# bastienjacquet/CudaDepthMapIntegration

Hardware: AMD Instinct MI355X
Metric: Gvoxel-projections/s (higher is better)
Workload: dtype f64

## Files before the change

### cudadepthmapintegration_amd/csrc/fusion_tile.hip

```cpp
#include <stdlib.h>

#include <algorithm>
#include <type_traits>

#include "fusion_kernels.h"
#include "fusion_device.h"

#ifndef DMI_T1_CHAINS
#define DMI_T1_CHAINS 4
#endif
#ifndef DMI_T1_COLUMN_CHAINS
#define DMI_T1_COLUMN_CHAINS 2
#endif
#if !defined(DMI_TUNING) && (defined(DMI_EXP_SKIP_WINDOW_VIEWS) || defined(DMI_EXP_SAME_REC) || defined(DMI_EXP_NO_WINDOW_LOADS) || \
                             defined(DMI_EXP_NO_LANE_MARGIN))
#error "a DMI_EXP_* switch that changes results was defined without DMI_TUNING"
#endif

namespace dmi {

int tile_shape_index(int variant);

namespace {

// ... 586 lines not shown
          f32x2 v;
          v.x = __uint_as_float(R[q]);
          v.y = __uint_as_float(R[q + 1]);
          asm volatile("" : "+v"(v));
          return v;
        };
        const f32x2 Bwi = pk_fnma_slo(O, pair_of(8), vec_of(2));
        const f32x2 Bwj = pk_fnma_slo(O, pair_of(10), vec_of(4));
        const f32x2 DH = pk_fnma_slo(O, pair_of(12), vec_of(6));
#ifdef DMI_WINPAIR_LANE_HELD
        const f32x2 H0 = pk_fma_hi0_vv(LJ, Bwj, pk_fma_lo0_vs(LJ, Bwi, A2));
#else
        const f32x2 H0 = pk_fma_hi0_vv(LJ, Bwj, pk_fma_lo0_vv(LJ, Bwi, A2));
#endif
        f32x2 CA;
        CA.x = acz;
        CA.y = __builtin_fmaf(acz, __uint_as_float(R[15]), -__uint_as_float(R[14]));
        const f32x2 C0 = pk_fma_hi0_sv(LJ, pair_of(10), pk_fma_lo0_sv(LJ, pair_of(8), CA));
        const f32x2 DC = vec_of(12);
        unsigned long long M2 = (0x4B400000ull + (unsigned)kWinAnchorX) | ((0x4B400000ull + (unsigned)kWinAnchorY) << 32);
        asm volatile("" : "+s"(M2));
        float magic_v = 0x1.8p23f + (float)(4 * kWinAnchorY);
        asm volatile("" : "+v"(magic_v));
        auto first_voxel = [&](double &hxf, double &hyf, double &czf64) __attribute__((always_inline)) {
          const kernarg_t kf = KFRESH();
          const TileMapRec *rf = kf->tile_maps + m;
          double wxf = wx, wyf = wy, wzf = wz0;
          if constexpr (ROT) {
            const czvec4 b = cload(reinterpret_cast<const czvec4 *>(kf->cz_table + (int64_t)k0 * 4));
            wxf = (wx + b[0]) + kf->g[3], wyf = (wy + b[1]) + kf->g[7], wzf = (wz0 + b[2]) + kf->g[11];
            czf64 = ((cload(&rf->rz0) * wxf + cload(&rf->rz1) * wyf) + cload(&kf->maps[m].rt[10]) * wzf) + cload(&rf->rz3);
          } else {
            czf64 = ((cload(&rf->rz0) * wx + cload(&rf->rz1) * wy) + cload(kf->cz_table + (int64_t)m * kf->kpad + k0)) + cload(&rf->rz3);
          }
          hxf = __builtin_fma(cload(&rf->cpx), wxf, __builtin_fma(cload(&rf->cpy), wyf, __builtin_fma(cload(&rf->cpz), wzf, cload(&rf->cp0))));
          hyf = __builtin_fma(cload(&rf->cqx), wxf, __builtin_fma(cload(&rf->cqy), wyf, __builtin_fma(cload(&rf->cqz), wzf, cload(&rf->cq0))));
        };
        uint32_t undecided = 0, und_kk = 0;
        uint32_t window = 0;
        constexpr int WG = 4;
#ifdef DMI_T1_RCP_EVERY_VOXEL
        constexpr bool kNewton = false;
#else
        constexpr bool kNewton = true;
#endif
        [[maybe_unused]] f32x2 r_below;
        uint32_t pw[WG], pc[WG];
        auto consume = [&](int g0) __attribute__((always_inline)) {
          __builtin_amdgcn_s_waitcnt(0xc07f);
          if ((und_kk >> g0) & ((1u << WG) - 1u)) {
  #pragma unroll
            for (int q = 0; q < WG; ++q) pw[q] &= ((undecided >> (g0 + q)) & 1u) - 1u;
          }
  #pragma unroll
          for (int q = 0; q < WG; ++q) {
            int mbit;
            asm("v_bfe_i32 %0, %1, %2, 1" : "=v"(mbit) : "v"(pw[q]), "v"(pc[q]));
            acc_fma_vs<BASE, TK>(g0 + q, __hiloint2double(mbit & 0x3ff00000, 0), free_space);
          }
        };
  #pragma unroll
        for (int g0 = 0; g0 < TK; g0 += WG) {
          uint32_t wg[WG], cg[WG];
          mask_t m_und[WG];
          constexpr int IL = DMI_T1_CHAINS;
          if constexpr (kNewton) {
            static_assert(WG == 4, "the link order below is written for groups of four");
            f32x2 h[WG], cth[WG], r[WG], rpm[WG], rp[WG], t[WG];
            float tw[WG], mx[WG];
            auto kbits = [](int kk) __attribute__((always_inline)) { return (unsigned long long)(unsigned)__float_as_int((float)kk); };
            auto lz = [&](int u) __attribute__((always_inline)) { cth[u] = g0 + u > 0 ? ordered::pk_fma_s(kbits(g0 + u), DC, C0) : C0; };
            auto lh = [&](int u) __attribute__((always_inline)) { h[u] = g0 + u > 0 ? ordered::pk_fma_s(kbits(g0 + u), DH, H0) : H0; };
            auto l2 = [&](int u) __attribute__((always_inline)) {
              if (g0 + u > 0) tw[u] = ordered::two_minus(cth[u].x, u > 0 ? r[u > 0 ? u - 1 : 0].x : r_below.x);
            };
            auto lr = [&](int u) __attribute__((always_inline)) {
              r[u].x = g0 + u > 0 ? ordered::mul(u > 0 ? r[u > 0 ? u - 1 : 0].x : r_below.x, tw[u]) : ordered::rcp(cth[u].x);
            };
            auto lq = [&](int u) __attribute__((always_inline)) { rpm[u] = ordered::pk_fma_lo_s(h[u], r[u], M2); };
            auto lp = [&](int u) __attribute__((always_inline)) { rp[u] = ordered::pk_sub_s(rpm[u], M2); };
            auto lt = [&](int u) __attribute__((always_inline)) { t[u] = ordered::pk_fnma_lo(rp[u], cth[u], h[u]); };
            auto lm = [&](int u) __attribute__((always_inline)) { mx[u] = ordered::max_abs(t[u].x, t[u].y); };
            lz(0), lz(1), lz(2), lz(3);
            l2(0), lh(0), lr(0), lh(1), l2(1), lh(2), lr(1), lq(0), l2(2), lp(0), lr(2), lq(1), l2(3), lt(0), lr(3), lh(3);
            lp(1), lq(2), lm(0), lq(3), lt(1), lp(2), lm(1), lp(3), lt(2), lt(3), lm(2), lm(3);
            r_below = r[WG - 1];
  #pragma unroll
            for (int u = 0; u < WG; ++u) {
              m_und[u] = ballot(!(mx[u] < cth[u].y));
// ... 41 lines not shown
          if (m_und_any) {
  #pragma unroll
            for (int q = 0; q < WG; ++q) {
              if (m_und[q]) {
                or_where(undecided, m_und[q], 1u << (g0 + q));
                und_kk |= 1u << (g0 + q);
              }
            }
          }
          if (g0 == 0)
            window = __builtin_amdgcn_alignbit(w_hi, w_lo, (unsigned)x0p & 31u);
          else
            consume(g0 - WG);
  #pragma unroll
          for (int q = 0; q < WG; ++q) {
            pw[q] = (uint32_t)__builtin_amdgcn_ds_bpermute((int)wg[q], (int)window);
            pc[q] = cg[q];
          }
        }
        consume(TK - WG);
#ifndef DMI_NO_WINREC_PREFETCH
        asm volatile("s_waitcnt lgkmcnt(0)" : "+s"(next_rec));
#endif
#pragma unroll 1
        while (und_kk) {
#ifdef DMI_TUNING
          ++dbg_redo;
          ++dbg_win_redo;
#endif
          const int kk = __builtin_ctz(und_kk);
          und_kk &= und_kk - 1;
          const bool mine = (undecided >> kk) & 1u;
          const kernarg_t k2 = KFRESH();
          const TileMapRec *r2 = k2->tile_maps + m;
          double hxf, hyf, czf64;
          first_voxel(hxf, hyf, czf64);
          const double kd = (double)kk;
          const double hxk = __builtin_fma(kd, cload(&r2->cdhx), hxf), hyk = __builtin_fma(kd, cload(&r2->cdhy), hyf);
          double cz2;
          if constexpr (ROT) {
            const czvec4 b = cload(reinterpret_cast<const czvec4 *>(k2->cz_table + (int64_t)(k0 + kk) * 4));
            const double wxk = (wx + b[0]) + k2->g[3], wyk = (wy + b[1]) + k2->g[7], wzk = (wz0 + b[2]) + k2->g[11];
            cz2 = ((cload(&r2->rz0) * wxk + cload(&r2->rz1) * wyk) + cload(&k2->maps[m].rt[10]) * wzk) + cload(&r2->rz3);
          } else {
            cz2 = ((cload(&r2->rz0) * wx + cload(&r2->rz1) * wy) + cload(k2->cz_table + (int64_t)m * k2->kpad + k0 + kk)) + cload(&r2->rz3);
          }
// ... 5 lines not shown
          const double fu = ua2 - ru2, fv = va2 - rv2;
          const double chk = __builtin_fma(cload(&r2->cerrk), r, __builtin_fmax(__builtin_fabs(fu), __builtin_fabs(fv)));
          const bool p2 = mine && chk < 0.5 && __builtin_fabs(e0) < tiny;
          const int col = cvt_saturating(ru2) - x0c, row = cvt_saturating(rv2) - y0c;
          const uint32_t word = (uint32_t)__builtin_amdgcn_ds_bpermute(row << 2, (int)window);
          double val = free_space;
          bool hit = p2 && ((word >> (col & 31)) & 1u);
          const bool exact = mine && !p2;
          if (ballot(exact)) {
            const __amdgpu_buffer_rsrc_t rsrc =
                __builtin_amdgcn_make_buffer_rsrc(const_cast<void *>(cload(&r2->depth)), (short)0, k2->depth_bytes, 0x00020000);
            double ev = 0.0;
            const bool eh = exact ? tile_exact<DepthT>(KC(full), m, rsrc, i, j, k0 + kk, ev) : false;
            if (exact) {
              hit = eh;
              val = ev;
            }
          }
#pragma unroll
          for (int q = 0; q < TK; ++q) {
            if (kk == q) acc_add_v<BASE, TK>(q, ballot(hit), val);
          }
        }
        continue;
      }
    }
    const kernarg_t kv = KFRESH();
    const TileMapRec *rec = kv->tile_maps + m;
    const double *ct = kv->cz_table + (int64_t)m * kv->kpad + k0;
    double sz, rz3, hx, hy;
    [[maybe_unused]] f32x2 H0 = {0.f, 0.f}, C0 = {0.f, 0.f}, DH = {0.f, 0.f}, DC = {0.f, 0.f};
    double r20 = 0, r21 = 0, r22 = 0;
    [[maybe_unused]] double cz_first = 0, wxf = wx, wyf = wy, wzf = wz0;
    if constexpr (ROT) {
      sz = lane_ok ? cload(&rec->rz3) : -__builtin_inf();
      rz3 = 0;
      hx = hy = 0;
      if constexpr (T1) {
        const czvec4 b = cload(reinterpret_cast<const czvec4 *>(kv->cz_table + (int64_t)k0 * 4));
        wxf = (wx + b[0]) + KA(g)[3], wyf = (wy + b[1]) + KA(g)[7], wzf = (wz0 + b[2]) + KA(g)[11];
        cz_first = ((cload(&rec->rz0) * wxf + cload(&rec->rz1) * wyf) + cload(&kv->maps[m].rt[10]) * wzf) + sz;
      } else {
        r20 = cload(&rec->rz0);
        r21 = cload(&rec->rz1);
        r22 = cload(&kv->maps[m].rt[10]);
      }
// ... 652 lines not shown
```

### cudadepthmapintegration_amd/csrc/fusion_tile_acc.inc

```

template <int BASE, int TK>
__device__ __forceinline__ void acc_add_s(const int kk, mask_t m, double v ) {
  mask_t saved;
  switch (BASE + 2 * kk) {
    case 64: if constexpr (64 >= BASE && 64 < BASE + 2 * TK) asm volatile("s_and_saveexec_b64 %0, %1\n\tv_add_f64 v[64:65], v[64:65], %2\n\ts_mov_b64 exec, %0" : "=&s"(saved) : "s"(m), "s"(v) : "v64", "v65", "scc"); break;
    case 66: if constexpr (66 >= BASE && 66 < BASE + 2 * TK) asm volatile("s_and_saveexec_b64 %0, %1\n\tv_add_f64 v[66:67], v[66:67], %2\n\ts_mov_b64 exec, %0" : "=&s"(saved) : "s"(m), "s"(v) : "v66", "v67", "scc"); break;
    case 68: if constexpr (68 >= BASE && 68 < BASE + 2 * TK) asm volatile("s_and_saveexec_b64 %0, %1\n\tv_add_f64 v[68:69], v[68:69], %2\n\ts_mov_b64 exec, %0" : "=&s"(saved) : "s"(m), "s"(v) : "v68", "v69", "scc"); break;
    case 70: if constexpr (70 >= BASE && 70 < BASE + 2 * TK) asm volatile("s_and_saveexec_b64 %0, %1\n\tv_add_f64 v[70:71], v[70:71], %2\n\ts_mov_b64 exec, %0" : "=&s"(saved) : "s"(m), "s"(v) : "v70", "v71", "scc"); break;
    case 72: if constexpr (72 >= BASE && 72 < BASE + 2 * TK) asm volatile("s_and_saveexec_b64 %0, %1\n\tv_add_f64 v[72:73], v[72:73], %2\n\ts_mov_b64 exec, %0" : "=&s"(saved) : "s"(m), "s"(v) : "v72", "v73", "scc"); break;
    case 74: if constexpr (74 >= BASE && 74 < BASE + 2 * TK) asm volatile("s_and_saveexec_b64 %0, %1\n\tv_add_f64 v[74:75], v[74:75], %2\n\ts_mov_b64 exec, %0" : "=&s"(saved) : "s"(m), "s"(v) : "v74", "v75", "scc"); break;
    case 76: if constexpr (76 >= BASE && 76 < BASE + 2 * TK) asm volatile("s_and_saveexec_b64 %0, %1\n\tv_add_f64 v[76:77], v[76:77], %2\n\ts_mov_b64 exec, %0" : "=&s"(saved) : "s"(m), "s"(v) : "v76", "v77", "scc"); break;
    case 78: if constexpr (78 >= BASE && 78 < BASE + 2 * TK) asm volatile("s_and_saveexec_b64 %0, %1\n\tv_add_f64 v[78:79], v[78:79], %2\n\ts_mov_b64 exec, %0" : "=&s"(saved) : "s"(m), "s"(v) : "v78", "v79", "scc"); break;
    case 80: if constexpr (80 >= BASE && 80 < BASE + 2 * TK) asm volatile("s_and_saveexec_b64 %0, %1\n\tv_add_f64 v[80:81], v[80:81], %2\n\ts_mov_b64 exec, %0" : "=&s"(saved) : "s"(m), "s"(v) : "v80", "v81", "scc"); break;
    case 82: if constexpr (82 >= BASE && 82 < BASE + 2 * TK) asm volatile("s_and_saveexec_b64 %0, %1\n\tv_add_f64 v[82:83], v[82:83], %2\n\ts_mov_b64 exec, %0" : "=&s"(saved) : "s"(m), "s"(v) : "v82", "v83", "scc"); break;
    case 84: if constexpr (84 >= BASE && 84 < BASE + 2 * TK) asm volatile("s_and_saveexec_b64 %0, %1\n\tv_add_f64 v[84:85], v[84:85], %2\n\ts_mov_b64 exec, %0" : "=&s"(saved) : "s"(m), "s"(v) : "v84", "v85", "scc"); break;
    case 86: if constexpr (86 >= BASE && 86 < BASE + 2 * TK) asm volatile("s_and_saveexec_b64 %0, %1\n\tv_add_f64 v[86:87], v[86:87], %2\n\ts_mov_b64 exec, %0" : "=&s"(saved) : "s"(m), "s"(v) : "v86", "v87", "scc"); break;
    case 88: if constexpr (88 >= BASE && 88 < BASE + 2 * TK) asm volatile("s_and_saveexec_b64 %0, %1\n\tv_add_f64 v[88:89], v[88:89], %2\n\ts_mov_b64 exec, %0" : "=&s"(saved) : "s"(m), "s"(v) : "v88", "v89", "scc"); break;
    case 90: if constexpr (90 >= BASE && 90 < BASE + 2 * TK) asm volatile("s_and_saveexec_b64 %0, %1\n\tv_add_f64 v[90:91], v[90:91], %2\n\ts_mov_b64 exec, %0" : "=&s"(saved) : "s"(m), "s"(v) : "v90", "v91", "scc"); break;
    case 92: if constexpr (92 >= BASE && 92 < BASE + 2 * TK) asm volatile("s_and_saveexec_b64 %0, %1\n\tv_add_f64 v[92:93], v[92:93], %2\n\ts_mov_b64 exec, %0" : "=&s"(saved) : "s"(m), "s"(v) : "v92", "v93", "scc"); break;
    case 94: if constexpr (94 >= BASE && 94 < BASE + 2 * TK) asm volatile("s_and_saveexec_b64 %0, %1\n\tv_add_f64 v[94:95], v[94:95], %2\n\ts_mov_b64 exec, %0" : "=&s"(saved) : "s"(m), "s"(v) : "v94", "v95", "scc"); break;
    case 96: if constexpr (96 >= BASE && 96 < BASE + 2 * TK) asm volatile("s_and_saveexec_b64 %0, %1\n\tv_add_f64 v[96:97], v[96:97], %2\n\ts_mov_b64 exec, %0" : "=&s"(saved) : "s"(m), "s"(v) : "v96", "v97", "scc"); break;
    case 98: if constexpr (98 >= BASE && 98 < BASE + 2 * TK) asm volatile("s_and_saveexec_b64 %0, %1\n\tv_add_f64 v[98:99], v[98:99], %2\n\ts_mov_b64 exec, %0" : "=&s"(saved) : "s"(m), "s"(v) : "v98", "v99", "scc"); break;
    case 100: if constexpr (100 >= BASE && 100 < BASE + 2 * TK) asm volatile("s_and_saveexec_b64 %0, %1\n\tv_add_f64 v[100:101], v[100:101], %2\n\ts_mov_b64 exec, %0" : "=&s"(saved) : "s"(m), "s"(v) : "v100", "v101", "scc"); break;
    case 102: if constexpr (102 >= BASE && 102 < BASE + 2 * TK) asm volatile("s_and_saveexec_b64 %0, %1\n\tv_add_f64 v[102:103], v[102:103], %2\n\ts_mov_b64 exec, %0" : "=&s"(saved) : "s"(m), "s"(v) : "v102", "v103", "scc"); break;
// ... 720 lines not shown
    case 154: if constexpr (154 >= BASE && 154 < BASE + 2 * TK) asm volatile("s_mov_b64 %[sx], exec\n\tv_add_f64 %[diff], %[cz], -%[d]\n\ts_mov_b64 %[sh], exec\n\tv_cmpx_lt_f64_e64 vcc, %[diff], -%[delta]\n\tv_add_f64 v[154:155], v[154:155], %[fs]\n\ts_mov_b64 exec, %[sh]\n\tv_cmpx_ngt_f64_e64 vcc, |%[diff]|, %[delta]\n\ts_cbranch_execz .Ldmi_pot_end_%=\n\tv_mul_f64 %[near], %[slope], %[diff]\n\ts_mov_b64 %[sh], exec\n\tv_cmpx_gt_f64_e64 vcc, %[diff], %[thick]\n\tv_mul_f64 %[near], %[rho], 1.0\n\ts_mov_b64 exec, %[sh]\n\tv_cmpx_lt_f64_e64 vcc, %[diff], -%[thick]\n\tv_mul_f64 %[near], %[rho], -1.0\n\ts_mov_b64 exec, %[sh]\n\tv_add_f64 v[154:155], v[154:155], %[near]\n\t.Ldmi_pot_end_%=:\n\ts_mov_b64 exec, %[sx]" : [diff] "=&v"(diff), [near] "=&v"(near), [sx] "=&s"(sx), [sh] "=&s"(sh) : [d] "v"(d), [cz] "v"(cz), [delta] "v"(delta), [thick] "v"(thick), [slope] "v"(slope), [fs] "s"(free_space), [rho] "s"(rho) : "v154", "v155", "vcc"); break;
    case 156: if constexpr (156 >= BASE && 156 < BASE + 2 * TK) asm volatile("s_mov_b64 %[sx], exec\n\tv_add_f64 %[diff], %[cz], -%[d]\n\ts_mov_b64 %[sh], exec\n\tv_cmpx_lt_f64_e64 vcc, %[diff], -%[delta]\n\tv_add_f64 v[156:157], v[156:157], %[fs]\n\ts_mov_b64 exec, %[sh]\n\tv_cmpx_ngt_f64_e64 vcc, |%[diff]|, %[delta]\n\ts_cbranch_execz .Ldmi_pot_end_%=\n\tv_mul_f64 %[near], %[slope], %[diff]\n\ts_mov_b64 %[sh], exec\n\tv_cmpx_gt_f64_e64 vcc, %[diff], %[thick]\n\tv_mul_f64 %[near], %[rho], 1.0\n\ts_mov_b64 exec, %[sh]\n\tv_cmpx_lt_f64_e64 vcc, %[diff], -%[thick]\n\tv_mul_f64 %[near], %[rho], -1.0\n\ts_mov_b64 exec, %[sh]\n\tv_add_f64 v[156:157], v[156:157], %[near]\n\t.Ldmi_pot_end_%=:\n\ts_mov_b64 exec, %[sx]" : [diff] "=&v"(diff), [near] "=&v"(near), [sx] "=&s"(sx), [sh] "=&s"(sh) : [d] "v"(d), [cz] "v"(cz), [delta] "v"(delta), [thick] "v"(thick), [slope] "v"(slope), [fs] "s"(free_space), [rho] "s"(rho) : "v156", "v157", "vcc"); break;
    case 158: if constexpr (158 >= BASE && 158 < BASE + 2 * TK) asm volatile("s_mov_b64 %[sx], exec\n\tv_add_f64 %[diff], %[cz], -%[d]\n\ts_mov_b64 %[sh], exec\n\tv_cmpx_lt_f64_e64 vcc, %[diff], -%[delta]\n\tv_add_f64 v[158:159], v[158:159], %[fs]\n\ts_mov_b64 exec, %[sh]\n\tv_cmpx_ngt_f64_e64 vcc, |%[diff]|, %[delta]\n\ts_cbranch_execz .Ldmi_pot_end_%=\n\tv_mul_f64 %[near], %[slope], %[diff]\n\ts_mov_b64 %[sh], exec\n\tv_cmpx_gt_f64_e64 vcc, %[diff], %[thick]\n\tv_mul_f64 %[near], %[rho], 1.0\n\ts_mov_b64 exec, %[sh]\n\tv_cmpx_lt_f64_e64 vcc, %[diff], -%[thick]\n\tv_mul_f64 %[near], %[rho], -1.0\n\ts_mov_b64 exec, %[sh]\n\tv_add_f64 v[158:159], v[158:159], %[near]\n\t.Ldmi_pot_end_%=:\n\ts_mov_b64 exec, %[sx]" : [diff] "=&v"(diff), [near] "=&v"(near), [sx] "=&s"(sx), [sh] "=&s"(sh) : [d] "v"(d), [cz] "v"(cz), [delta] "v"(delta), [thick] "v"(thick), [slope] "v"(slope), [fs] "s"(free_space), [rho] "s"(rho) : "v158", "v159", "vcc"); break;
    case 160: if constexpr (160 >= BASE && 160 < BASE + 2 * TK) asm volatile("s_mov_b64 %[sx], exec\n\tv_add_f64 %[diff], %[cz], -%[d]\n\ts_mov_b64 %[sh], exec\n\tv_cmpx_lt_f64_e64 vcc, %[diff], -%[delta]\n\tv_add_f64 v[160:161], v[160:161], %[fs]\n\ts_mov_b64 exec, %[sh]\n\tv_cmpx_ngt_f64_e64 vcc, |%[diff]|, %[delta]\n\ts_cbranch_execz .Ldmi_pot_end_%=\n\tv_mul_f64 %[near], %[slope], %[diff]\n\ts_mov_b64 %[sh], exec\n\tv_cmpx_gt_f64_e64 vcc, %[diff], %[thick]\n\tv_mul_f64 %[near], %[rho], 1.0\n\ts_mov_b64 exec, %[sh]\n\tv_cmpx_lt_f64_e64 vcc, %[diff], -%[thick]\n\tv_mul_f64 %[near], %[rho], -1.0\n\ts_mov_b64 exec, %[sh]\n\tv_add_f64 v[160:161], v[160:161], %[near]\n\t.Ldmi_pot_end_%=:\n\ts_mov_b64 exec, %[sx]" : [diff] "=&v"(diff), [near] "=&v"(near), [sx] "=&s"(sx), [sh] "=&s"(sh) : [d] "v"(d), [cz] "v"(cz), [delta] "v"(delta), [thick] "v"(thick), [slope] "v"(slope), [fs] "s"(free_space), [rho] "s"(rho) : "v160", "v161", "vcc"); break;
    case 162: if constexpr (162 >= BASE && 162 < BASE + 2 * TK) asm volatile("s_mov_b64 %[sx], exec\n\tv_add_f64 %[diff], %[cz], -%[d]\n\ts_mov_b64 %[sh], exec\n\tv_cmpx_lt_f64_e64 vcc, %[diff], -%[delta]\n\tv_add_f64 v[162:163], v[162:163], %[fs]\n\ts_mov_b64 exec, %[sh]\n\tv_cmpx_ngt_f64_e64 vcc, |%[diff]|, %[delta]\n\ts_cbranch_execz .Ldmi_pot_end_%=\n\tv_mul_f64 %[near], %[slope], %[diff]\n\ts_mov_b64 %[sh], exec\n\tv_cmpx_gt_f64_e64 vcc, %[diff], %[thick]\n\tv_mul_f64 %[near], %[rho], 1.0\n\ts_mov_b64 exec, %[sh]\n\tv_cmpx_lt_f64_e64 vcc, %[diff], -%[thick]\n\tv_mul_f64 %[near], %[rho], -1.0\n\ts_mov_b64 exec, %[sh]\n\tv_add_f64 v[162:163], v[162:163], %[near]\n\t.Ldmi_pot_end_%=:\n\ts_mov_b64 exec, %[sx]" : [diff] "=&v"(diff), [near] "=&v"(near), [sx] "=&s"(sx), [sh] "=&s"(sh) : [d] "v"(d), [cz] "v"(cz), [delta] "v"(delta), [thick] "v"(thick), [slope] "v"(slope), [fs] "s"(free_space), [rho] "s"(rho) : "v162", "v163", "vcc"); break;
    case 164: if constexpr (164 >= BASE && 164 < BASE + 2 * TK) asm volatile("s_mov_b64 %[sx], exec\n\tv_add_f64 %[diff], %[cz], -%[d]\n\ts_mov_b64 %[sh], exec\n\tv_cmpx_lt_f64_e64 vcc, %[diff], -%[delta]\n\tv_add_f64 v[164:165], v[164:165], %[fs]\n\ts_mov_b64 exec, %[sh]\n\tv_cmpx_ngt_f64_e64 vcc, |%[diff]|, %[delta]\n\ts_cbranch_execz .Ldmi_pot_end_%=\n\tv_mul_f64 %[near], %[slope], %[diff]\n\ts_mov_b64 %[sh], exec\n\tv_cmpx_gt_f64_e64 vcc, %[diff], %[thick]\n\tv_mul_f64 %[near], %[rho], 1.0\n\ts_mov_b64 exec, %[sh]\n\tv_cmpx_lt_f64_e64 vcc, %[diff], -%[thick]\n\tv_mul_f64 %[near], %[rho], -1.0\n\ts_mov_b64 exec, %[sh]\n\tv_add_f64 v[164:165], v[164:165], %[near]\n\t.Ldmi_pot_end_%=:\n\ts_mov_b64 exec, %[sx]" : [diff] "=&v"(diff), [near] "=&v"(near), [sx] "=&s"(sx), [sh] "=&s"(sh) : [d] "v"(d), [cz] "v"(cz), [delta] "v"(delta), [thick] "v"(thick), [slope] "v"(slope), [fs] "s"(free_space), [rho] "s"(rho) : "v164", "v165", "vcc"); break;
    case 166: if constexpr (166 >= BASE && 166 < BASE + 2 * TK) asm volatile("s_mov_b64 %[sx], exec\n\tv_add_f64 %[diff], %[cz], -%[d]\n\ts_mov_b64 %[sh], exec\n\tv_cmpx_lt_f64_e64 vcc, %[diff], -%[delta]\n\tv_add_f64 v[166:167], v[166:167], %[fs]\n\ts_mov_b64 exec, %[sh]\n\tv_cmpx_ngt_f64_e64 vcc, |%[diff]|, %[delta]\n\ts_cbranch_execz .Ldmi_pot_end_%=\n\tv_mul_f64 %[near], %[slope], %[diff]\n\ts_mov_b64 %[sh], exec\n\tv_cmpx_gt_f64_e64 vcc, %[diff], %[thick]\n\tv_mul_f64 %[near], %[rho], 1.0\n\ts_mov_b64 exec, %[sh]\n\tv_cmpx_lt_f64_e64 vcc, %[diff], -%[thick]\n\tv_mul_f64 %[near], %[rho], -1.0\n\ts_mov_b64 exec, %[sh]\n\tv_add_f64 v[166:167], v[166:167], %[near]\n\t.Ldmi_pot_end_%=:\n\ts_mov_b64 exec, %[sx]" : [diff] "=&v"(diff), [near] "=&v"(near), [sx] "=&s"(sx), [sh] "=&s"(sh) : [d] "v"(d), [cz] "v"(cz), [delta] "v"(delta), [thick] "v"(thick), [slope] "v"(slope), [fs] "s"(free_space), [rho] "s"(rho) : "v166", "v167", "vcc"); break;
    case 168: if constexpr (168 >= BASE && 168 < BASE + 2 * TK) asm volatile("s_mov_b64 %[sx], exec\n\tv_add_f64 %[diff], %[cz], -%[d]\n\ts_mov_b64 %[sh], exec\n\tv_cmpx_lt_f64_e64 vcc, %[diff], -%[delta]\n\tv_add_f64 v[168:169], v[168:169], %[fs]\n\ts_mov_b64 exec, %[sh]\n\tv_cmpx_ngt_f64_e64 vcc, |%[diff]|, %[delta]\n\ts_cbranch_execz .Ldmi_pot_end_%=\n\tv_mul_f64 %[near], %[slope], %[diff]\n\ts_mov_b64 %[sh], exec\n\tv_cmpx_gt_f64_e64 vcc, %[diff], %[thick]\n\tv_mul_f64 %[near], %[rho], 1.0\n\ts_mov_b64 exec, %[sh]\n\tv_cmpx_lt_f64_e64 vcc, %[diff], -%[thick]\n\tv_mul_f64 %[near], %[rho], -1.0\n\ts_mov_b64 exec, %[sh]\n\tv_add_f64 v[168:169], v[168:169], %[near]\n\t.Ldmi_pot_end_%=:\n\ts_mov_b64 exec, %[sx]" : [diff] "=&v"(diff), [near] "=&v"(near), [sx] "=&s"(sx), [sh] "=&s"(sh) : [d] "v"(d), [cz] "v"(cz), [delta] "v"(delta), [thick] "v"(thick), [slope] "v"(slope), [fs] "s"(free_space), [rho] "s"(rho) : "v168", "v169", "vcc"); break;
    case 170: if constexpr (170 >= BASE && 170 < BASE + 2 * TK) asm volatile("s_mov_b64 %[sx], exec\n\tv_add_f64 %[diff], %[cz], -%[d]\n\ts_mov_b64 %[sh], exec\n\tv_cmpx_lt_f64_e64 vcc, %[diff], -%[delta]\n\tv_add_f64 v[170:171], v[170:171], %[fs]\n\ts_mov_b64 exec, %[sh]\n\tv_cmpx_ngt_f64_e64 vcc, |%[diff]|, %[delta]\n\ts_cbranch_execz .Ldmi_pot_end_%=\n\tv_mul_f64 %[near], %[slope], %[diff]\n\ts_mov_b64 %[sh], exec\n\tv_cmpx_gt_f64_e64 vcc, %[diff], %[thick]\n\tv_mul_f64 %[near], %[rho], 1.0\n\ts_mov_b64 exec, %[sh]\n\tv_cmpx_lt_f64_e64 vcc, %[diff], -%[thick]\n\tv_mul_f64 %[near], %[rho], -1.0\n\ts_mov_b64 exec, %[sh]\n\tv_add_f64 v[170:171], v[170:171], %[near]\n\t.Ldmi_pot_end_%=:\n\ts_mov_b64 exec, %[sx]" : [diff] "=&v"(diff), [near] "=&v"(near), [sx] "=&s"(sx), [sh] "=&s"(sh) : [d] "v"(d), [cz] "v"(cz), [delta] "v"(delta), [thick] "v"(thick), [slope] "v"(slope), [fs] "s"(free_space), [rho] "s"(rho) : "v170", "v171", "vcc"); break;
    case 172: if constexpr (172 >= BASE && 172 < BASE + 2 * TK) asm volatile("s_mov_b64 %[sx], exec\n\tv_add_f64 %[diff], %[cz], -%[d]\n\ts_mov_b64 %[sh], exec\n\tv_cmpx_lt_f64_e64 vcc, %[diff], -%[delta]\n\tv_add_f64 v[172:173], v[172:173], %[fs]\n\ts_mov_b64 exec, %[sh]\n\tv_cmpx_ngt_f64_e64 vcc, |%[diff]|, %[delta]\n\ts_cbranch_execz .Ldmi_pot_end_%=\n\tv_mul_f64 %[near], %[slope], %[diff]\n\ts_mov_b64 %[sh], exec\n\tv_cmpx_gt_f64_e64 vcc, %[diff], %[thick]\n\tv_mul_f64 %[near], %[rho], 1.0\n\ts_mov_b64 exec, %[sh]\n\tv_cmpx_lt_f64_e64 vcc, %[diff], -%[thick]\n\tv_mul_f64 %[near], %[rho], -1.0\n\ts_mov_b64 exec, %[sh]\n\tv_add_f64 v[172:173], v[172:173], %[near]\n\t.Ldmi_pot_end_%=:\n\ts_mov_b64 exec, %[sx]" : [diff] "=&v"(diff), [near] "=&v"(near), [sx] "=&s"(sx), [sh] "=&s"(sh) : [d] "v"(d), [cz] "v"(cz), [delta] "v"(delta), [thick] "v"(thick), [slope] "v"(slope), [fs] "s"(free_space), [rho] "s"(rho) : "v172", "v173", "vcc"); break;
    case 174: if constexpr (174 >= BASE && 174 < BASE + 2 * TK) asm volatile("s_mov_b64 %[sx], exec\n\tv_add_f64 %[diff], %[cz], -%[d]\n\ts_mov_b64 %[sh], exec\n\tv_cmpx_lt_f64_e64 vcc, %[diff], -%[delta]\n\tv_add_f64 v[174:175], v[174:175], %[fs]\n\ts_mov_b64 exec, %[sh]\n\tv_cmpx_ngt_f64_e64 vcc, |%[diff]|, %[delta]\n\ts_cbranch_execz .Ldmi_pot_end_%=\n\tv_mul_f64 %[near], %[slope], %[diff]\n\ts_mov_b64 %[sh], exec\n\tv_cmpx_gt_f64_e64 vcc, %[diff], %[thick]\n\tv_mul_f64 %[near], %[rho], 1.0\n\ts_mov_b64 exec, %[sh]\n\tv_cmpx_lt_f64_e64 vcc, %[diff], -%[thick]\n\tv_mul_f64 %[near], %[rho], -1.0\n\ts_mov_b64 exec, %[sh]\n\tv_add_f64 v[174:175], v[174:175], %[near]\n\t.Ldmi_pot_end_%=:\n\ts_mov_b64 exec, %[sx]" : [diff] "=&v"(diff), [near] "=&v"(near), [sx] "=&s"(sx), [sh] "=&s"(sh) : [d] "v"(d), [cz] "v"(cz), [delta] "v"(delta), [thick] "v"(thick), [slope] "v"(slope), [fs] "s"(free_space), [rho] "s"(rho) : "v174", "v175", "vcc"); break;
    case 176: if constexpr (176 >= BASE && 176 < BASE + 2 * TK) asm volatile("s_mov_b64 %[sx], exec\n\tv_add_f64 %[diff], %[cz], -%[d]\n\ts_mov_b64 %[sh], exec\n\tv_cmpx_lt_f64_e64 vcc, %[diff], -%[delta]\n\tv_add_f64 v[176:177], v[176:177], %[fs]\n\ts_mov_b64 exec, %[sh]\n\tv_cmpx_ngt_f64_e64 vcc, |%[diff]|, %[delta]\n\ts_cbranch_execz .Ldmi_pot_end_%=\n\tv_mul_f64 %[near], %[slope], %[diff]\n\ts_mov_b64 %[sh], exec\n\tv_cmpx_gt_f64_e64 vcc, %[diff], %[thick]\n\tv_mul_f64 %[near], %[rho], 1.0\n\ts_mov_b64 exec, %[sh]\n\tv_cmpx_lt_f64_e64 vcc, %[diff], -%[thick]\n\tv_mul_f64 %[near], %[rho], -1.0\n\ts_mov_b64 exec, %[sh]\n\tv_add_f64 v[176:177], v[176:177], %[near]\n\t.Ldmi_pot_end_%=:\n\ts_mov_b64 exec, %[sx]" : [diff] "=&v"(diff), [near] "=&v"(near), [sx] "=&s"(sx), [sh] "=&s"(sh) : [d] "v"(d), [cz] "v"(cz), [delta] "v"(delta), [thick] "v"(thick), [slope] "v"(slope), [fs] "s"(free_space), [rho] "s"(rho) : "v176", "v177", "vcc"); break;
    case 178: if constexpr (178 >= BASE && 178 < BASE + 2 * TK) asm volatile("s_mov_b64 %[sx], exec\n\tv_add_f64 %[diff], %[cz], -%[d]\n\ts_mov_b64 %[sh], exec\n\tv_cmpx_lt_f64_e64 vcc, %[diff], -%[delta]\n\tv_add_f64 v[178:179], v[178:179], %[fs]\n\ts_mov_b64 exec, %[sh]\n\tv_cmpx_ngt_f64_e64 vcc, |%[diff]|, %[delta]\n\ts_cbranch_execz .Ldmi_pot_end_%=\n\tv_mul_f64 %[near], %[slope], %[diff]\n\ts_mov_b64 %[sh], exec\n\tv_cmpx_gt_f64_e64 vcc, %[diff], %[thick]\n\tv_mul_f64 %[near], %[rho], 1.0\n\ts_mov_b64 exec, %[sh]\n\tv_cmpx_lt_f64_e64 vcc, %[diff], -%[thick]\n\tv_mul_f64 %[near], %[rho], -1.0\n\ts_mov_b64 exec, %[sh]\n\tv_add_f64 v[178:179], v[178:179], %[near]\n\t.Ldmi_pot_end_%=:\n\ts_mov_b64 exec, %[sx]" : [diff] "=&v"(diff), [near] "=&v"(near), [sx] "=&s"(sx), [sh] "=&s"(sh) : [d] "v"(d), [cz] "v"(cz), [delta] "v"(delta), [thick] "v"(thick), [slope] "v"(slope), [fs] "s"(free_space), [rho] "s"(rho) : "v178", "v179", "vcc"); break;
    case 180: if constexpr (180 >= BASE && 180 < BASE + 2 * TK) asm volatile("s_mov_b64 %[sx], exec\n\tv_add_f64 %[diff], %[cz], -%[d]\n\ts_mov_b64 %[sh], exec\n\tv_cmpx_lt_f64_e64 vcc, %[diff], -%[delta]\n\tv_add_f64 v[180:181], v[180:181], %[fs]\n\ts_mov_b64 exec, %[sh]\n\tv_cmpx_ngt_f64_e64 vcc, |%[diff]|, %[delta]\n\ts_cbranch_execz .Ldmi_pot_end_%=\n\tv_mul_f64 %[near], %[slope], %[diff]\n\ts_mov_b64 %[sh], exec\n\tv_cmpx_gt_f64_e64 vcc, %[diff], %[thick]\n\tv_mul_f64 %[near], %[rho], 1.0\n\ts_mov_b64 exec, %[sh]\n\tv_cmpx_lt_f64_e64 vcc, %[diff], -%[thick]\n\tv_mul_f64 %[near], %[rho], -1.0\n\ts_mov_b64 exec, %[sh]\n\tv_add_f64 v[180:181], v[180:181], %[near]\n\t.Ldmi_pot_end_%=:\n\ts_mov_b64 exec, %[sx]" : [diff] "=&v"(diff), [near] "=&v"(near), [sx] "=&s"(sx), [sh] "=&s"(sh) : [d] "v"(d), [cz] "v"(cz), [delta] "v"(delta), [thick] "v"(thick), [slope] "v"(slope), [fs] "s"(free_space), [rho] "s"(rho) : "v180", "v181", "vcc"); break;
    case 182: if constexpr (182 >= BASE && 182 < BASE + 2 * TK) asm volatile("s_mov_b64 %[sx], exec\n\tv_add_f64 %[diff], %[cz], -%[d]\n\ts_mov_b64 %[sh], exec\n\tv_cmpx_lt_f64_e64 vcc, %[diff], -%[delta]\n\tv_add_f64 v[182:183], v[182:183], %[fs]\n\ts_mov_b64 exec, %[sh]\n\tv_cmpx_ngt_f64_e64 vcc, |%[diff]|, %[delta]\n\ts_cbranch_execz .Ldmi_pot_end_%=\n\tv_mul_f64 %[near], %[slope], %[diff]\n\ts_mov_b64 %[sh], exec\n\tv_cmpx_gt_f64_e64 vcc, %[diff], %[thick]\n\tv_mul_f64 %[near], %[rho], 1.0\n\ts_mov_b64 exec, %[sh]\n\tv_cmpx_lt_f64_e64 vcc, %[diff], -%[thick]\n\tv_mul_f64 %[near], %[rho], -1.0\n\ts_mov_b64 exec, %[sh]\n\tv_add_f64 v[182:183], v[182:183], %[near]\n\t.Ldmi_pot_end_%=:\n\ts_mov_b64 exec, %[sx]" : [diff] "=&v"(diff), [near] "=&v"(near), [sx] "=&s"(sx), [sh] "=&s"(sh) : [d] "v"(d), [cz] "v"(cz), [delta] "v"(delta), [thick] "v"(thick), [slope] "v"(slope), [fs] "s"(free_space), [rho] "s"(rho) : "v182", "v183", "vcc"); break;
    case 184: if constexpr (184 >= BASE && 184 < BASE + 2 * TK) asm volatile("s_mov_b64 %[sx], exec\n\tv_add_f64 %[diff], %[cz], -%[d]\n\ts_mov_b64 %[sh], exec\n\tv_cmpx_lt_f64_e64 vcc, %[diff], -%[delta]\n\tv_add_f64 v[184:185], v[184:185], %[fs]\n\ts_mov_b64 exec, %[sh]\n\tv_cmpx_ngt_f64_e64 vcc, |%[diff]|, %[delta]\n\ts_cbranch_execz .Ldmi_pot_end_%=\n\tv_mul_f64 %[near], %[slope], %[diff]\n\ts_mov_b64 %[sh], exec\n\tv_cmpx_gt_f64_e64 vcc, %[diff], %[thick]\n\tv_mul_f64 %[near], %[rho], 1.0\n\ts_mov_b64 exec, %[sh]\n\tv_cmpx_lt_f64_e64 vcc, %[diff], -%[thick]\n\tv_mul_f64 %[near], %[rho], -1.0\n\ts_mov_b64 exec, %[sh]\n\tv_add_f64 v[184:185], v[184:185], %[near]\n\t.Ldmi_pot_end_%=:\n\ts_mov_b64 exec, %[sx]" : [diff] "=&v"(diff), [near] "=&v"(near), [sx] "=&s"(sx), [sh] "=&s"(sh) : [d] "v"(d), [cz] "v"(cz), [delta] "v"(delta), [thick] "v"(thick), [slope] "v"(slope), [fs] "s"(free_space), [rho] "s"(rho) : "v184", "v185", "vcc"); break;
    case 186: if constexpr (186 >= BASE && 186 < BASE + 2 * TK) asm volatile("s_mov_b64 %[sx], exec\n\tv_add_f64 %[diff], %[cz], -%[d]\n\ts_mov_b64 %[sh], exec\n\tv_cmpx_lt_f64_e64 vcc, %[diff], -%[delta]\n\tv_add_f64 v[186:187], v[186:187], %[fs]\n\ts_mov_b64 exec, %[sh]\n\tv_cmpx_ngt_f64_e64 vcc, |%[diff]|, %[delta]\n\ts_cbranch_execz .Ldmi_pot_end_%=\n\tv_mul_f64 %[near], %[slope], %[diff]\n\ts_mov_b64 %[sh], exec\n\tv_cmpx_gt_f64_e64 vcc, %[diff], %[thick]\n\tv_mul_f64 %[near], %[rho], 1.0\n\ts_mov_b64 exec, %[sh]\n\tv_cmpx_lt_f64_e64 vcc, %[diff], -%[thick]\n\tv_mul_f64 %[near], %[rho], -1.0\n\ts_mov_b64 exec, %[sh]\n\tv_add_f64 v[186:187], v[186:187], %[near]\n\t.Ldmi_pot_end_%=:\n\ts_mov_b64 exec, %[sx]" : [diff] "=&v"(diff), [near] "=&v"(near), [sx] "=&s"(sx), [sh] "=&s"(sh) : [d] "v"(d), [cz] "v"(cz), [delta] "v"(delta), [thick] "v"(thick), [slope] "v"(slope), [fs] "s"(free_space), [rho] "s"(rho) : "v186", "v187", "vcc"); break;
    case 188: if constexpr (188 >= BASE && 188 < BASE + 2 * TK) asm volatile("s_mov_b64 %[sx], exec\n\tv_add_f64 %[diff], %[cz], -%[d]\n\ts_mov_b64 %[sh], exec\n\tv_cmpx_lt_f64_e64 vcc, %[diff], -%[delta]\n\tv_add_f64 v[188:189], v[188:189], %[fs]\n\ts_mov_b64 exec, %[sh]\n\tv_cmpx_ngt_f64_e64 vcc, |%[diff]|, %[delta]\n\ts_cbranch_execz .Ldmi_pot_end_%=\n\tv_mul_f64 %[near], %[slope], %[diff]\n\ts_mov_b64 %[sh], exec\n\tv_cmpx_gt_f64_e64 vcc, %[diff], %[thick]\n\tv_mul_f64 %[near], %[rho], 1.0\n\ts_mov_b64 exec, %[sh]\n\tv_cmpx_lt_f64_e64 vcc, %[diff], -%[thick]\n\tv_mul_f64 %[near], %[rho], -1.0\n\ts_mov_b64 exec, %[sh]\n\tv_add_f64 v[188:189], v[188:189], %[near]\n\t.Ldmi_pot_end_%=:\n\ts_mov_b64 exec, %[sx]" : [diff] "=&v"(diff), [near] "=&v"(near), [sx] "=&s"(sx), [sh] "=&s"(sh) : [d] "v"(d), [cz] "v"(cz), [delta] "v"(delta), [thick] "v"(thick), [slope] "v"(slope), [fs] "s"(free_space), [rho] "s"(rho) : "v188", "v189", "vcc"); break;
    case 190: if constexpr (190 >= BASE && 190 < BASE + 2 * TK) asm volatile("s_mov_b64 %[sx], exec\n\tv_add_f64 %[diff], %[cz], -%[d]\n\ts_mov_b64 %[sh], exec\n\tv_cmpx_lt_f64_e64 vcc, %[diff], -%[delta]\n\tv_add_f64 v[190:191], v[190:191], %[fs]\n\ts_mov_b64 exec, %[sh]\n\tv_cmpx_ngt_f64_e64 vcc, |%[diff]|, %[delta]\n\ts_cbranch_execz .Ldmi_pot_end_%=\n\tv_mul_f64 %[near], %[slope], %[diff]\n\ts_mov_b64 %[sh], exec\n\tv_cmpx_gt_f64_e64 vcc, %[diff], %[thick]\n\tv_mul_f64 %[near], %[rho], 1.0\n\ts_mov_b64 exec, %[sh]\n\tv_cmpx_lt_f64_e64 vcc, %[diff], -%[thick]\n\tv_mul_f64 %[near], %[rho], -1.0\n\ts_mov_b64 exec, %[sh]\n\tv_add_f64 v[190:191], v[190:191], %[near]\n\t.Ldmi_pot_end_%=:\n\ts_mov_b64 exec, %[sx]" : [diff] "=&v"(diff), [near] "=&v"(near), [sx] "=&s"(sx), [sh] "=&s"(sh) : [d] "v"(d), [cz] "v"(cz), [delta] "v"(delta), [thick] "v"(thick), [slope] "v"(slope), [fs] "s"(free_space), [rho] "s"(rho) : "v190", "v191", "vcc"); break;
    default: break;
  }
}

template <int BASE, int TK>
__device__ __forceinline__ double acc_get(const int kk) {
  double v = 0.0;
  switch (BASE + 2 * kk) {
    case 64: if constexpr (64 >= BASE && 64 < BASE + 2 * TK) asm volatile("v_mov_b64 %0, v[64:65]" : "=v"(v)); break;
    case 66: if constexpr (66 >= BASE && 66 < BASE + 2 * TK) asm volatile("v_mov_b64 %0, v[66:67]" : "=v"(v)); break;
    case 68: if constexpr (68 >= BASE && 68 < BASE + 2 * TK) asm volatile("v_mov_b64 %0, v[68:69]" : "=v"(v)); break;
    case 70: if constexpr (70 >= BASE && 70 < BASE + 2 * TK) asm volatile("v_mov_b64 %0, v[70:71]" : "=v"(v)); break;
    case 72: if constexpr (72 >= BASE && 72 < BASE + 2 * TK) asm volatile("v_mov_b64 %0, v[72:73]" : "=v"(v)); break;
    case 74: if constexpr (74 >= BASE && 74 < BASE + 2 * TK) asm volatile("v_mov_b64 %0, v[74:75]" : "=v"(v)); break;
    case 76: if constexpr (76 >= BASE && 76 < BASE + 2 * TK) asm volatile("v_mov_b64 %0, v[76:77]" : "=v"(v)); break;
    case 78: if constexpr (78 >= BASE && 78 < BASE + 2 * TK) asm volatile("v_mov_b64 %0, v[78:79]" : "=v"(v)); break;
    case 80: if constexpr (80 >= BASE && 80 < BASE + 2 * TK) asm volatile("v_mov_b64 %0, v[80:81]" : "=v"(v)); break;
    case 82: if constexpr (82 >= BASE && 82 < BASE + 2 * TK) asm volatile("v_mov_b64 %0, v[82:83]" : "=v"(v)); break;
    case 84: if constexpr (84 >= BASE && 84 < BASE + 2 * TK) asm volatile("v_mov_b64 %0, v[84:85]" : "=v"(v)); break;
    case 86: if constexpr (86 >= BASE && 86 < BASE + 2 * TK) asm volatile("v_mov_b64 %0, v[86:87]" : "=v"(v)); break;
    case 88: if constexpr (88 >= BASE && 88 < BASE + 2 * TK) asm volatile("v_mov_b64 %0, v[88:89]" : "=v"(v)); break;
    case 90: if constexpr (90 >= BASE && 90 < BASE + 2 * TK) asm volatile("v_mov_b64 %0, v[90:91]" : "=v"(v)); break;
    case 92: if constexpr (92 >= BASE && 92 < BASE + 2 * TK) asm volatile("v_mov_b64 %0, v[92:93]" : "=v"(v)); break;
    case 94: if constexpr (94 >= BASE && 94 < BASE + 2 * TK) asm volatile("v_mov_b64 %0, v[94:95]" : "=v"(v)); break;
    case 96: if constexpr (96 >= BASE && 96 < BASE + 2 * TK) asm volatile("v_mov_b64 %0, v[96:97]" : "=v"(v)); break;
    case 98: if constexpr (98 >= BASE && 98 < BASE + 2 * TK) asm volatile("v_mov_b64 %0, v[98:99]" : "=v"(v)); break;
    case 100: if constexpr (100 >= BASE && 100 < BASE + 2 * TK) asm volatile("v_mov_b64 %0, v[100:101]" : "=v"(v)); break;
// ... 50 lines not shown
```

Before: 3156.

## Hand-schedule window group links in asm and hoist redo-loop record loads

For 16-voxel window tiles, the per-group Newton reciprocal and projection chain is replaced by one hand-scheduled inline-asm block with fixed register assignments. The block interleaves four voxels' packed FMA, reciprocal-refinement and max steps to hide latency and avoid compiler spills. The redo loop for undecided voxels now loads the tile map record once as vector scalar loads before the loop, instead of reloading fields and recomputing the first voxel every iteration. The cost is fragile hard-coded register usage (v40-v61) that could clash with compiler allocation, plus a layout static_assert tying the code to TileMapRec.

```diff
diff --git a/cudadepthmapintegration_amd/csrc/fusion_tile.hip b/cudadepthmapintegration_amd/csrc/fusion_tile.hip
--- a/cudadepthmapintegration_amd/csrc/fusion_tile.hip
+++ b/cudadepthmapintegration_amd/csrc/fusion_tile.hip
@@ -632,6 +632,7 @@
         asm volatile("" : "+s"(M2));
         float magic_v = 0x1.8p23f + (float)(4 * kWinAnchorY);
         asm volatile("" : "+v"(magic_v));
+#ifdef DMI_WIN_REDO_LOADS_IN_LOOP
         auto first_voxel = [&](double &hxf, double &hyf, double &czf64) __attribute__((always_inline)) {
           const kernarg_t kf = KFRESH();
           const TileMapRec *rf = kf->tile_maps + m;
@@ -646,6 +647,7 @@
           hxf = __builtin_fma(cload(&rf->cpx), wxf, __builtin_fma(cload(&rf->cpy), wyf, __builtin_fma(cload(&rf->cpz), wzf, cload(&rf->cp0))));
           hyf = __builtin_fma(cload(&rf->cqx), wxf, __builtin_fma(cload(&rf->cqy), wyf, __builtin_fma(cload(&rf->cqz), wzf, cload(&rf->cq0))));
         };
+#endif
         uint32_t undecided = 0, und_kk = 0;
         uint32_t window = 0;
         constexpr int WG = 4;
@@ -654,7 +656,13 @@
 #else
         constexpr bool kNewton = true;
 #endif
+#if defined(DMI_WIN_GROUP_LINKS) || defined(DMI_T1_RCP_EVERY_VOXEL)
+        constexpr bool kGroupAsm = false;
+#else
+        constexpr bool kGroupAsm = TK == 16;
+#endif
         [[maybe_unused]] f32x2 r_below;
+        [[maybe_unused]] float r_below_asm;
         uint32_t pw[WG], pc[WG];
         auto consume = [&](int g0) __attribute__((always_inline)) {
           __builtin_amdgcn_s_waitcnt(0xc07f);
@@ -674,7 +682,16 @@
           uint32_t wg[WG], cg[WG];
           mask_t m_und[WG];
           constexpr int IL = DMI_T1_CHAINS;
-          if constexpr (kNewton) {
+          if constexpr (kGroupAsm) {
+            f32x2 rpm[WG];
+            float mx[WG], thr[WG];
+            win_group4<BASE>(g0, H0, DH, C0, DC, M2, magic_v, r_below_asm, rpm, mx, thr, wg);
+  #pragma unroll
+            for (int u = 0; u < WG; ++u) {
+              m_und[u] = ballot(!(mx[u] < thr[u]));
+              cg[u] = (uint32_t)__float_as_int(rpm[u].x);
+            }
+          } else if constexpr (kNewton) {
             static_assert(WG == 4, "the link order below is written for groups of four");
             f32x2 h[WG], cth[WG], r[WG], rpm[WG], rp[WG], t[WG];
             float tw[WG], mx[WG];
@@ -762,6 +779,7 @@
 #ifndef DMI_NO_WINREC_PREFETCH
         asm volatile("s_waitcnt lgkmcnt(0)" : "+s"(next_rec));
 #endif
+#ifdef DMI_WIN_REDO_LOADS_IN_LOOP
 #pragma unroll 1
         while (und_kk) {
 #ifdef DMI_TUNING
@@ -813,6 +831,90 @@
             if (kk == q) acc_add_v<BASE, TK>(q, ballot(hit), val);
           }
         }
+#else
+        auto redo_voxel = [&](int kk, double hxk, double hyk, double cz2, double cerrk) __attribute__((always_inline)) {
+          const bool mine = (undecided >> kk) & 1u;
+          const double r0 = __builtin_amdgcn_rcp(cz2);
+          const double e0 = __builtin_fma(-cz2, r0, 1.0);
+          const double r = __builtin_fma(r0, e0, r0);
+          const double ua2 = hxk * r, va2 = hyk * r;
+          const double ru2 = __builtin_rint(ua2), rv2 = __builtin_rint(va2);
+          const double fu = ua2 - ru2, fv = va2 - rv2;
+          const double chk = __builtin_fma(cerrk, r, __builtin_fmax(__builtin_fabs(fu), __builtin_fabs(fv)));
+          const bool p2 = mine && chk < 0.5 && __builtin_fabs(e0) < tiny;
+          const int col = cvt_saturating(ru2) - x0c, row = cvt_saturating(rv2) - y0c;
+          const uint32_t word = (uint32_t)__builtin_amdgcn_ds_bpermute(row << 2, (int)window);
+          double val = free_space;
+          bool hit = p2 && ((word >> (col & 31)) & 1u);
+          const bool exact = mine && !p2;
+          if (ballot(exact)) {
+            const kernarg_t ke = KFRESH();
+            const __amdgpu_buffer_rsrc_t rsrc =
+                __builtin_amdgcn_make_buffer_rsrc(const_cast<void *>(cload(&(ke->tile_maps + m)->depth)), (short)0, ke->depth_bytes, 0x00020000);
+            double ev = 0.0;
+            const bool eh = exact ? tile_exact<DepthT>(KC(full), m, rsrc, i, j, k0 + kk, ev) : false;
+            if (exact) {
+              hit = eh;
+              val = ev;
+            }
+          }
+#pragma unroll
+          for (int q = 0; q < TK; ++q) {
+            if (kk == q) acc_add_v<BASE, TK>(q, ballot(hit), val);
+          }
+        };
+        if (und_kk) {
+          typedef double rec4 __attribute__((ext_vector_type(4), aligned(8)));
+          typedef double rec8 __attribute__((ext_vector_type(8), aligned(8)));
+          const kernarg_t k2 = KFRESH();
+          const TileMapRec *r2 = k2->tile_maps + m;
+          const rec8 cp = *reinterpret_cast<const rec8 __attribute__((address_space(4))) *>(reinterpret_cast<uintptr_t>(&r2->cpx));
+          const rec4 cd = *reinterpret_cast<const rec4 __attribute__((address_space(4))) *>(reinterpret_cast<uintptr_t>(&r2->cdhx));
+          const rec4 rz = *reinterpret_cast<const rec4 __attribute__((address_space(4))) *>(reinterpret_cast<uintptr_t>(&r2->rz0));
+          constexpr size_t oc = offsetof(TileMapRec, cpx), od = offsetof(TileMapRec, cdhx);
+          static_assert(offsetof(TileMapRec, cpy) == oc + 8 && offsetof(TileMapRec, cpz) == oc + 16 && offsetof(TileMapRec, cp0) == oc + 24 &&
+                            offsetof(TileMapRec, cqx) == oc + 32 && offsetof(TileMapRec, cqy) == oc + 40 && offsetof(TileMapRec, cqz) == oc + 48 &&
+                            offsetof(TileMapRec, cq0) == oc + 56 && offsetof(TileMapRec, cdhy) == od + 8 && offsetof(TileMapRec, cerrk) == od + 16 &&
+                            od + 32 <= sizeof(TileMapRec) && offsetof(TileMapRec, rz0) == 0 && offsetof(TileMapRec, rz1) == 8 &&
+                            offsetof(TileMapRec, rz3) == 16,
+                        "the redo reads these fields of TileMapRec as three vectors: every one where the vector's element is");
+          [[maybe_unused]] double gx = 0, gy = 0, gz = 0, r22 = 0, sz2 = 0;
+          [[maybe_unused]] const double *cz_row = nullptr;
+          double wxf = wx, wyf = wy, wzf = wz0;
+          if constexpr (ROT) {
+            gx = k2->g[3], gy = k2->g[7], gz = k2->g[11];
+            r22 = cload(&k2->maps[m].rt[10]);
+            cz_row = k2->cz_table + (int64_t)k0 * 4;
+            const czvec4 b = cload(reinterpret_cast<const czvec4 *>(cz_row));
+            wxf = (wx + b[0]) + gx, wyf = (wy + b[1]) + gy, wzf = (wz0 + b[2]) + gz;
+          } else {
+            cz_row = k2->cz_table + (int64_t)m * k2->kpad + k0;
+            sz2 = rz[0] * wx + rz[1] * wy;
+          }
+          const double hxf = __builtin_fma(cp[0], wxf, __builtin_fma(cp[1], wyf, __builtin_fma(cp[2], wzf, cp[3])));
+          const double hyf = __builtin_fma(cp[4], wxf, __builtin_fma(cp[5], wyf, __builtin_fma(cp[6], wzf, cp[7])));
+#pragma unroll 1
+          do {
+#ifdef DMI_TUNING
+            ++dbg_redo;
+            ++dbg_win_redo;
+#endif
+            const int kk = __builtin_ctz(und_kk);
+            und_kk &= und_kk - 1;
+            const double kd = (double)kk;
+            const double hxk = __builtin_fma(kd, cd[0], hxf), hyk = __builtin_fma(kd, cd[1], hyf);
+            double cz2;
+            if constexpr (ROT) {
+              const czvec4 b = cload(reinterpret_cast<const czvec4 *>(cz_row + (int64_t)kk * 4));
+              const double wxk = (wx + b[0]) + gx, wyk = (wy + b[1]) + gy, wzk = (wz0 + b[2]) + gz;
+              cz2 = ((rz[0] * wxk + rz[1] * wyk) + r22 * wzk) + rz[2];
+            } else {
+              cz2 = (sz2 + cload(cz_row + kk)) + rz[2];
+            }
+            redo_voxel(kk, hxk, hyk, cz2, cd[2]);
+          } while (und_kk);
+        }
+#endif
         continue;
       }
     }
diff --git a/cudadepthmapintegration_amd/csrc/fusion_tile_acc.inc b/cudadepthmapintegration_amd/csrc/fusion_tile_acc.inc
--- a/cudadepthmapintegration_amd/csrc/fusion_tile_acc.inc
+++ b/cudadepthmapintegration_amd/csrc/fusion_tile_acc.inc
@@ -766,6 +766,23 @@
   }
 }
 
+typedef float win_f32x2 __attribute__((ext_vector_type(2)));
+template <int BASE>
+__device__ __forceinline__ void win_group4(const int g0, win_f32x2 H0, win_f32x2 DH, win_f32x2 C0, win_f32x2 DC, unsigned long long M2, float magic_v,
+                                           float &r_below, win_f32x2 (&rpm)[4], float (&mx)[4], float (&thr)[4], unsigned (&wg)[4]) {
+  static_assert(BASE == 96, "win_group4 is generated for the 16-voxel WIN instantiations (the 8-voxel ones spill more with it)");
+  unsigned long long kbits[4];
+  for (int u = 0; u < 4; ++u) kbits[u] = (unsigned long long)__builtin_bit_cast(unsigned, (float)(g0 + u));
+  if constexpr (BASE == 96) {
+    if (g0 == 0) {
+      thr[0] = C0.y;
+      asm volatile("v_pk_fma_f32 v[42:43], %[k1], %[DC], %[C0] op_sel_hi:[0,1,1]\n\tv_pk_fma_f32 v[44:45], %[k2], %[DC], %[C0] op_sel_hi:[0,1,1]\n\tv_pk_fma_f32 v[46:47], %[k3], %[DC], %[C0] op_sel_hi:[0,1,1]\n\tv_rcp_f32 v48, %[c0x]\n\tv_pk_fma_f32 v[58:59], %[k1], %[DH], %[H0] op_sel_hi:[0,1,1]\n\tv_fma_f32 v51, -v42, v48, 2.0\n\tv_pk_fma_f32 v[60:61], %[k2], %[DH], %[H0] op_sel_hi:[0,1,1]\n\tv_mul_f32 v50, v48, v51\n\tv_pk_fma_f32 %[q0], %[H0], v[48:49], %[M2] op_sel_hi:[1,0,1]\n\tv_fma_f32 v53, -v44, v50, 2.0\n\tv_pk_add_f32 v[48:49], %[q0], %[M2] neg_lo:[0,1] neg_hi:[0,1]\n\tv_mul_f32 v52, v50, v53\n\tv_pk_fma_f32 %[q1], v[58:59], v[50:51], %[M2] op_sel_hi:[1,0,1]\n\tv_fma_f32 v55, -v46, v52, 2.0\n\tv_pk_fma_f32 v[56:57], v[48:49], %[C0], %[H0] op_sel_hi:[1,0,1] neg_lo:[1,0,0] neg_hi:[1,0,0]\n\tv_mul_f32 v54, v52, v55\n\tv_fma_f32 %[a0], 4.0, v49, %[magic]\n\tv_pk_add_f32 v[50:51], %[q1], %[M2] neg_lo:[0,1] neg_hi:[0,1]\n\tv_pk_fma_f32 %[q2], v[60:61], v[52:53], %[M2] op_sel_hi:[1,0,1]\n\tv_pk_fma_f32 v[58:59], v[50:51], v[42:43], v[58:59] op_sel_hi:[1,0,1] neg_lo:[1,0,0] neg_hi:[1,0,0]\n\tv_pk_add_f32 v[52:53], %[q2], %[M2] neg_lo:[0,1] neg_hi:[0,1]\n\tv_fma_f32 %[a1], 4.0, v51, %[magic]\n\tv_max_f32 v50, |v56|, |v57|\n\tv_pk_fma_f32 v[56:57], %[k3], %[DH], %[H0] op_sel_hi:[0,1,1]\n\tv_max_f32 v51, |v58|, |v59|\n\tv_pk_fma_f32 v[60:61], v[52:53], v[44:45], v[60:61] op_sel_hi:[1,0,1] neg_lo:[1,0,0] neg_hi:[1,0,0]\n\tv_fma_f32 %[a2], 4.0, v53, %[magic]\n\tv_pk_fma_f32 %[q3], v[56:57], v[54:55], %[M2] op_sel_hi:[1,0,1]\n\tv_pk_add_f32 v[48:49], %[q3], %[M2] neg_lo:[0,1] neg_hi:[0,1]\n\tv_max_f32 v52, |v60|, |v61|\n\tv_pk_fma_f32 v[56:57], v[48:49], v[46:47], v[56:57] op_sel_hi:[1,0,1] neg_lo:[1,0,0] neg_hi:[1,0,0]\n\tv_fma_f32 %[a3], 4.0, v49, %[magic]\n\tv_max_f32 v53, |v56|, |v57|" : "=&{v54}"(r_below), [q0] "=&v"(rpm[0]), "=&{v50}"(mx[0]), [a0] "=&v"(wg[0]), [q1] "=&v"(rpm[1]), "=&{v51}"(mx[1]), [a1] "=&v"(wg[1]), "=&{v43}"(thr[1]), [q2] "=&v"(rpm[2]), "=&{v52}"(mx[2]), [a2] "=&v"(wg[2]), "=&{v45}"(thr[2]), [q3] "=&v"(rpm[3]), "=&{v53}"(mx[3]), [a3] "=&v"(wg[3]), "=&{v47}"(thr[3]) : [H0] "v"(H0), [DH] "v"(DH), [C0] "v"(C0), [DC] "v"(DC), [M2] "s"(M2), [magic] "v"(magic_v), [c0x] "v"(C0.x), [k1] "s"(kbits[1]), [k2] "s"(kbits[2]), [k3] "s"(kbits[3]) : "v40", "v41", "v42", "v44", "v46", "v48", "v49", "v55", "v56", "v57", "v58", "v59", "v60", "v61");
+    } else {
+      asm volatile("v_pk_fma_f32 v[40:41], %[k0], %[DC], %[C0] op_sel_hi:[0,1,1]\n\tv_pk_fma_f32 v[42:43], %[k1], %[DC], %[C0] op_sel_hi:[0,1,1]\n\tv_pk_fma_f32 v[44:45], %[k2], %[DC], %[C0] op_sel_hi:[0,1,1]\n\tv_pk_fma_f32 v[46:47], %[k3], %[DC], %[C0] op_sel_hi:[0,1,1]\n\tv_fma_f32 v49, -v40, v54, 2.0\n\tv_pk_fma_f32 v[56:57], %[k0], %[DH], %[H0] op_sel_hi:[0,1,1]\n\tv_mul_f32 v48, v54, v49\n\tv_pk_fma_f32 v[58:59], %[k1], %[DH], %[H0] op_sel_hi:[0,1,1]\n\tv_fma_f32 v51, -v42, v48, 2.0\n\tv_pk_fma_f32 v[60:61], %[k2], %[DH], %[H0] op_sel_hi:[0,1,1]\n\tv_mul_f32 v50, v48, v51\n\tv_pk_fma_f32 %[q0], v[56:57], v[48:49], %[M2] op_sel_hi:[1,0,1]\n\tv_fma_f32 v53, -v44, v50, 2.0\n\tv_pk_add_f32 v[48:49], %[q0], %[M2] neg_lo:[0,1] neg_hi:[0,1]\n\tv_mul_f32 v52, v50, v53\n\tv_pk_fma_f32 %[q1], v[58:59], v[50:51], %[M2] op_sel_hi:[1,0,1]\n\tv_fma_f32 v55, -v46, v52, 2.0\n\tv_pk_fma_f32 v[56:57], v[48:49], v[40:41], v[56:57] op_sel_hi:[1,0,1] neg_lo:[1,0,0] neg_hi:[1,0,0]\n\tv_mul_f32 v54, v52, v55\n\tv_fma_f32 %[a0], 4.0, v49, %[magic]\n\tv_pk_add_f32 v[50:51], %[q1], %[M2] neg_lo:[0,1] neg_hi:[0,1]\n\tv_pk_fma_f32 %[q2], v[60:61], v[52:53], %[M2] op_sel_hi:[1,0,1]\n\tv_pk_fma_f32 v[58:59], v[50:51], v[42:43], v[58:59] op_sel_hi:[1,0,1] neg_lo:[1,0,0] neg_hi:[1,0,0]\n\tv_pk_add_f32 v[52:53], %[q2], %[M2] neg_lo:[0,1] neg_hi:[0,1]\n\tv_fma_f32 %[a1], 4.0, v51, %[magic]\n\tv_max_f32 v50, |v56|, |v57|\n\tv_pk_fma_f32 v[56:57], %[k3], %[DH], %[H0] op_sel_hi:[0,1,1]\n\tv_max_f32 v51, |v58|, |v59|\n\tv_pk_fma_f32 v[60:61], v[52:53], v[44:45], v[60:61] op_sel_hi:[1,0,1] neg_lo:[1,0,0] neg_hi:[1,0,0]\n\tv_fma_f32 %[a2], 4.0, v53, %[magic]\n\tv_pk_fma_f32 %[q3], v[56:57], v[54:55], %[M2] op_sel_hi:[1,0,1]\n\tv_pk_add_f32 v[48:49], %[q3], %[M2] neg_lo:[0,1] neg_hi:[0,1]\n\tv_max_f32 v52, |v60|, |v61|\n\tv_pk_fma_f32 v[56:57], v[48:49], v[46:47], v[56:57] op_sel_hi:[1,0,1] neg_lo:[1,0,0] neg_hi:[1,0,0]\n\tv_fma_f32 %[a3], 4.0, v49, %[magic]\n\tv_max_f32 v53, |v56|, |v57|" : "+{v54}"(r_below), [q0] "=&v"(rpm[0]), "=&{v50}"(mx[0]), [a0] "=&v"(wg[0]), "=&{v41}"(thr[0]), [q1] "=&v"(rpm[1]), "=&{v51}"(mx[1]), [a1] "=&v"(wg[1]), "=&{v43}"(thr[1]), [q2] "=&v"(rpm[2]), "=&{v52}"(mx[2]), [a2] "=&v"(wg[2]), "=&{v45}"(thr[2]), [q3] "=&v"(rpm[3]), "=&{v53}"(mx[3]), [a3] "=&v"(wg[3]), "=&{v47}"(thr[3]) : [H0] "v"(H0), [DH] "v"(DH), [C0] "v"(C0), [DC] "v"(DC), [M2] "s"(M2), [magic] "v"(magic_v), [k0] "s"(kbits[0]), [k1] "s"(kbits[1]), [k2] "s"(kbits[2]), [k3] "s"(kbits[3]) : "v40", "v42", "v44", "v46", "v48", "v49", "v55", "v56", "v57", "v58", "v59", "v60", "v61");
+    }
+  }
+}
+
 template <int BASE, int TK>
 __device__ __forceinline__ double acc_get(const int kk) {
   double v = 0.0;
```

New measurement: 3188, median of 6. 1.0% higher.
